# Artemarius/cuda-gaussian-splatting

Measured on AMD Instinct MI355X. Metric: fwd+bwd Mpixels/s @1080p, 1M Gaussians, SH3, higher is better.
Workload: dtype f32

## Files before the change

cuda-gaussian-splatting_amd/csrc/cugs_raster_common.h:

```cpp
#pragma once

#include "cugs_gaussian_math.h"
#include "cugs_blend_cull.h"

#include <type_traits>

#define CUGS_REC_F4 3

struct RasterGeom {
    int width, height, ntx, ntiles;
    float bg0, bg1, bg2;
};

struct RasterSrc {
    const int32_t* tile_ranges;
    const int32_t* gidx;
    const float* packed;
    const float* means_2d;
    const float* cov_2d_inv;
    const float* rgb;
    const float* opa;
    const uint4* tile_order;
};

template <typename F>
static inline void cugs_with_bool(bool flag, F&& f) {
    if (flag) f(std::true_type{});
    else f(std::false_type{});
}

__device__ __forceinline__ void cugs_stage_cull(const float4& r0, float4& r1, float tile_cx, float tile_cy) {
    r1.z = cugs_cull_limit(r0.x, r0.y, r0.z, r0.w, r1.x, r1.z, tile_cx, tile_cy);
}
__device__ __forceinline__ bool may_touch_quad(float4 r0, float4 r1, float qx0, float qy0,
                                               float wx, float wy) {
    return cugs_cull_may_touch(r0.x, r0.y, r0.z, r0.w, r1.x, r1.z, qx0, qy0, wx, wy);
}

template <bool PACKED, bool DEPTH = false>
__device__ __forceinline__ int stage_record(const RasterSrc& s, int li, int end, float4* s_rec, float tile_cx,
                                            float tile_cy, const float* __restrict__ depths = nullptr) {
    if (li >= end) return -1;
    const int g = s.gidx[li];
    float4 r0, r1, r2;
    if (PACKED) {
        const float4* src = reinterpret_cast<const float4*>(s.packed + (int64_t)g * CUGS_PACKED_STRIDE);
        r0 = src[0]; r1 = src[1]; r2 = src[2];
    } else {
        const float a = s.cov_2d_inv[g * 3 + 0], c = s.cov_2d_inv[g * 3 + 2], o = s.opa[g];
        r0 = make_float4(s.means_2d[g * 2 + 0], s.means_2d[g * 2 + 1], a, s.cov_2d_inv[g * 3 + 1]);
        r1 = make_float4(c, o, (o >= (1.0f / 255.0f)) ? logf(255.0f * o) : -1.0f, 0.0f);
        r2 = make_float4(s.rgb[g * 3 + 0], 0.0f, s.rgb[g * 3 + 1], s.rgb[g * 3 + 2]);
    }
    r1.w = __int_as_float(g);
    cugs_stage_cull(r0, r1, tile_cx, tile_cy);
    if (DEPTH) r2.y = depths[g];
    s_rec[threadIdx.x * CUGS_REC_F4 + 0] = r0;
    s_rec[threadIdx.x * CUGS_REC_F4 + 1] = r1;
    s_rec[threadIdx.x * CUGS_REC_F4 + 2] = r2;
    return g;
}

struct ActiveRect { float x0, y0, wx, wy; };
__device__ __forceinline__ ActiveRect active_rect(unsigned long long active, float quad_cx, float quad_cy) {
    unsigned cols = (unsigned)active | (unsigned)(active >> 32);
    cols |= cols >> 16;
    cols |= cols >> 8;
    cols &= 0xFFu;
    const int x0 = __builtin_ctz(cols), x1 = 31 - __builtin_clz(cols);
    const int y0 = __builtin_ctzll(active) >> 3, y1 = (63 - __builtin_clzll(active)) >> 3;
    return ActiveRect{quad_cx + (float)x0, quad_cy + (float)y0, (float)(x1 - x0), (float)(y1 - y0)};
}

#define CUGS_HIT_GROUP 4
__device__ __forceinline__ unsigned cugs_pop_hit_desc(unsigned long long& mask) {
    const unsigned bit = 63u - (unsigned)__builtin_clzll(mask);
    mask &= ~(1ull << bit);
    return bit;
}
__device__ __forceinline__ unsigned cugs_pop_hit_asc(unsigned long long& mask) {
    const unsigned bit = (unsigned)__builtin_ctzll(mask);
    mask &= mask - 1ull;
    return bit;
}
__device__ __forceinline__ unsigned long long cugs_pop_hits4_desc(unsigned long long& mask, unsigned rec_base) {
    const unsigned r0 = rec_base + cugs_pop_hit_desc(mask) * CUGS_REC_F4;
    const unsigned r1 = rec_base + cugs_pop_hit_desc(mask) * CUGS_REC_F4;
    const unsigned r2 = rec_base + cugs_pop_hit_desc(mask) * CUGS_REC_F4;
    const unsigned r3 = rec_base + cugs_pop_hit_desc(mask) * CUGS_REC_F4;
    return (unsigned long long)(r0 | (r1 << 16)) | ((unsigned long long)(r2 | (r3 << 16)) << 32);
}
__device__ __forceinline__ int cugs_hit(unsigned long long hitrecs, int field) {
    return (int)((hitrecs >> (16 * field)) & 0xFFFFull);
}
__device__ __forceinline__ unsigned long long cugs_set_hit(unsigned long long hitrecs, int field, unsigned rec) {
    return (hitrecs & ~(0xFFFFull << (16 * field))) | ((unsigned long long)rec << (16 * field));
}

struct PixelEval { float dx, dy, gx, gy, e; };
__device__ __forceinline__ float pixel_alpha_raw(float pxf, float pyf, float mx, float my, float a, float b,
                                                 float c, float o, float open, PixelEval& r) {
    r.dx = pxf - mx;
    r.dy = pyf - my;
    r.gx = fmaf(a, r.dx, b * r.dy);
    r.gy = fmaf(b, r.dx, c * r.dy);
    const float q = fmaf(r.dx, r.gx, r.dy * r.gy);
    r.e = cugs_blend_exp_q(q);
    const float gate = fmaf(q, 0x1p127f, 1.0f);
    return __builtin_fminf(__builtin_fminf((o * open) * r.e, 0.99f), gate);
}
__device__ __forceinline__ float pixel_alpha(float pxf, float pyf, float mx, float my, float a, float b,
                                             float c, float o, float open, PixelEval& r) {
    const float alpha = pixel_alpha_raw(pxf, pyf, mx, my, a, b, c, o, open, r);
    return (alpha < (1.0f / 255.0f)) ? 0.0f : alpha;
}


__device__ __forceinline__ float sat_fma(float a, float b, float c) {
    return __builtin_amdgcn_fmed3f(fmaf(a, b, c), 0.0f, 1.0f);
}
__device__ __forceinline__ float sat_add(float a, float b) { return __builtin_amdgcn_fmed3f(a + b, 0.0f, 1.0f); }
__device__ __forceinline__ float sat_mul(float a, float b) { return __builtin_amdgcn_fmed3f(a * b, 0.0f, 1.0f); }

#define CUGS_ALPHA_MIN_PRED 0x1.01010p-8f
__device__ __forceinline__ float passes_alpha_min(float x) {
    return sat_fma(x, 0x1p32f, -CUGS_ALPHA_MIN_PRED * 0x1p32f);
}
__device__ __forceinline__ float below_alpha_cap(float x) { return sat_fma(x, -0x1p32f, 0.99f * 0x1p32f); }

__device__ __forceinline__ int reduce9t_slot(int lane) {
    if (lane & 3) return -1;
    const int bank = (lane >> 2) & 3, row = lane >> 4;
    const int perm[4] = {0, 2, 1, 3};
    if (row == 0) return perm[bank];
    if (row == 1) return bank == 3 ? 8 : 4 + perm[bank];
    if (row == 2 && bank == 0) return 7;
    return -1;
}

__device__ __forceinline__ float reduce9t(float cA, float cB, float v2, float v3, float v4, float v5, float v6,
                                          float v8, float v7) {
    float a0, a1, a2, a3, a4, b0, b1, b2, d;
    asm volatile(
        "s_nop 1\n\t"
        "v_add_f32_dpp %0, %10, %9 row_mirror row_mask:0xf bank_mask:0xf\n\t"
        "v_add_f32_dpp %1, %11, %11 row_mirror row_mask:0xf bank_mask:0x3\n\t"
        "v_add_f32_dpp %1, %12, %12 row_mirror row_mask:0xf bank_mask:0xc\n\t"
        "v_add_f32_dpp %2, %13, %13 row_mirror row_mask:0xf bank_mask:0x3\n\t"
        "v_add_f32_dpp %2, %14, %14 row_mirror row_mask:0xf bank_mask:0xc\n\t"
        "v_add_f32_dpp %3, %15, %15 row_mirror row_mask:0xf bank_mask:0x3\n\t"
        "v_add_f32_dpp %3, %16, %16 row_mirror row_mask:0xf bank_mask:0xc\n\t"
        "v_add_f32_dpp %4, %17, %17 row_mirror row_mask:0xf bank_mask:0xf\n\t"
        "v_add_f32_dpp %5, %0, %0 row_half_mirror row_mask:0xf bank_mask:0x5\n\t"
        "v_add_f32_dpp %5, %1, %1 row_half_mirror row_mask:0xf bank_mask:0xa\n\t"
        "v_add_f32_dpp %7, %4, %4 row_half_mirror row_mask:0xf bank_mask:0xf\n\t"
        "v_add_f32_dpp %6, %2, %2 row_half_mirror row_mask:0xf bank_mask:0x5\n\t"
        "v_add_f32_dpp %6, %3, %3 row_half_mirror row_mask:0xf bank_mask:0xa\n\t"
        "v_mov_b32 %8, %7\n\t"
        "s_nop 1\n\t"
        "v_permlane16_swap_b32 %5, %6\n\t"
        "v_permlane16_swap_b32 %7, %8\n\t"
        "v_add_f32 %5, %5, %6\n\t"
        "v_add_f32 %7, %7, %8\n\t"
        "s_nop 1\n\t"
        "v_permlane32_swap_b32 %5, %7\n\t"
        "v_add_f32 %8, %5, %7\n\t"
        "s_nop 1\n\t"
        "v_add_f32_dpp %8, %8, %8 quad_perm:[1,0,3,2] row_mask:0xf bank_mask:0xf\n\t"
        "s_nop 1\n\t"
        "v_add_f32_dpp %8, %8, %8 quad_perm:[2,3,0,1] row_mask:0xf bank_mask:0xf\n\t"
        : "=&v"(a0), "=&v"(a1), "=&v"(a2), "=&v"(a3), "=&v"(a4), "=&v"(b0), "=&v"(b1), "=&v"(b2), "=&v"(d)
        : "v"(cA), "v"(cB), "v"(v2), "v"(v3), "v"(v4), "v"(v5), "v"(v6), "v"(v8), "v"(v7));
    return d;
}

template <int CTRL>
__device__ __forceinline__ float dpp_mov(float v) {
    return __builtin_bit_cast(float, __builtin_amdgcn_update_dpp(0, __builtin_bit_cast(int, v), CTRL, 0xF, 0xF, false));
}
template <int CTRL>
__device__ __forceinline__ float xchg_add(bool side, float a, float b) {
    return (side ? b : a) + dpp_mov<CTRL>(side ? a : b);
}

__device__ __forceinline__ int reduce9r16_slot(int lane) {
    const int r = lane & 15, bank = r >> 2;
    const int perm[4] = {0, 2, 1, 3};
    if ((r & 3) == 0) return perm[bank];
    if ((r & 3) == 2) return bank == 3 ? 8 : 4 + perm[bank];
    if (r == 1) return 7;
    return -1;
}

__device__ __forceinline__ float reduce_r16_tail(float b0, float b1, float b2, int lane) {
    const bool s1 = (lane & 2) != 0, s0 = (lane & 1) != 0;
    const float c0 = xchg_add<0x4E>(s1, b0, b1);
    const float c1 = b2 + dpp_mov<0x4E>(b2);
    return xchg_add<0xB1>(s0, c0, c1);
}

__device__ __forceinline__ float reduce9r16(float cA, float cB, float v2, float v3, float v4, float v5, float v6,
                                            float v8, float v7, int lane) {
    float a0, a1, a2, a3, a4, b0, b1, b2;
    asm volatile(
        "s_nop 1\n\t"
        "v_add_f32_dpp %0, %9, %8 row_mirror row_mask:0xf bank_mask:0xf\n\t"
        "v_add_f32_dpp %1, %10, %10 row_mirror row_mask:0xf bank_mask:0x3\n\t"
        "v_add_f32_dpp %1, %11, %11 row_mirror row_mask:0xf bank_mask:0xc\n\t"
        "v_add_f32_dpp %2, %12, %12 row_mirror row_mask:0xf bank_mask:0x3\n\t"
        "v_add_f32_dpp %2, %13, %13 row_mirror row_mask:0xf bank_mask:0xc\n\t"
        "v_add_f32_dpp %3, %14, %14 row_mirror row_mask:0xf bank_mask:0x3\n\t"
        "v_add_f32_dpp %3, %15, %15 row_mirror row_mask:0xf bank_mask:0xc\n\t"
        "v_add_f32_dpp %4, %16, %16 row_mirror row_mask:0xf bank_mask:0xf\n\t"
        "v_add_f32_dpp %5, %0, %0 row_half_mirror row_mask:0xf bank_mask:0x5\n\t"
        "v_add_f32_dpp %5, %1, %1 row_half_mirror row_mask:0xf bank_mask:0xa\n\t"
        "v_add_f32_dpp %7, %4, %4 row_half_mirror row_mask:0xf bank_mask:0xf\n\t"
        "v_add_f32_dpp %6, %2, %2 row_half_mirror row_mask:0xf bank_mask:0x5\n\t"
        "v_add_f32_dpp %6, %3, %3 row_half_mirror row_mask:0xf bank_mask:0xa\n\t"
        "s_nop 1\n\t"
        : "=&v"(a0), "=&v"(a1), "=&v"(a2), "=&v"(a3), "=&v"(a4), "=&v"(b0), "=&v"(b1), "=&v"(b2)
        : "v"(cA), "v"(cB), "v"(v2), "v"(v3), "v"(v4), "v"(v5), "v"(v6), "v"(v8), "v"(v7));
    return reduce_r16_tail(b0, b1, b2, lane);
}

__device__ __forceinline__ int reduce10r16_slot(int lane) {
    return ((lane & 15) == 9) ? 9 : reduce9r16_slot(lane);
}

__device__ __forceinline__ float reduce10r16(float cA, float cB, float v2, float v3, float v4, float v5, float v6,
                                             float v8, float v7, float v9, int lane) {
    float a0, a1, a2, a3, a4, b0, b1, b2;
    asm volatile(
        "s_nop 1\n\t"
        "v_add_f32_dpp %0, %9, %8 row_mirror row_mask:0xf bank_mask:0xf\n\t"
        "v_add_f32_dpp %1, %10, %10 row_mirror row_mask:0xf bank_mask:0x3\n\t"
        "v_add_f32_dpp %1, %11, %11 row_mirror row_mask:0xf bank_mask:0xc\n\t"
        "v_add_f32_dpp %2, %12, %12 row_mirror row_mask:0xf bank_mask:0x3\n\t"
        "v_add_f32_dpp %2, %13, %13 row_mirror row_mask:0xf bank_mask:0xc\n\t"
        "v_add_f32_dpp %3, %14, %14 row_mirror row_mask:0xf bank_mask:0x3\n\t"
        "v_add_f32_dpp %3, %15, %15 row_mirror row_mask:0xf bank_mask:0xc\n\t"
        "v_add_f32_dpp %4, %16, %16 row_mirror row_mask:0xf bank_mask:0x3\n\t"
        "v_add_f32_dpp %4, %17, %17 row_mirror row_mask:0xf bank_mask:0xc\n\t"
        "v_add_f32_dpp %5, %0, %0 row_half_mirror row_mask:0xf bank_mask:0x5\n\t"
        "v_add_f32_dpp %5, %1, %1 row_half_mirror row_mask:0xf bank_mask:0xa\n\t"
        "v_add_f32_dpp %7, %4, %4 row_half_mirror row_mask:0xf bank_mask:0xf\n\t"
        "v_add_f32_dpp %6, %2, %2 row_half_mirror row_mask:0xf bank_mask:0x5\n\t"
        "v_add_f32_dpp %6, %3, %3 row_half_mirror row_mask:0xf bank_mask:0xa\n\t"
        "s_nop 1\n\t"
        : "=&v"(a0), "=&v"(a1), "=&v"(a2), "=&v"(a3), "=&v"(a4), "=&v"(b0), "=&v"(b1), "=&v"(b2)
        : "v"(cA), "v"(cB), "v"(v2), "v"(v3), "v"(v4), "v"(v5), "v"(v6), "v"(v8), "v"(v7), "v"(v9));
    return reduce_r16_tail(b0, b1, b2, lane);
}

__device__ __forceinline__ int reduce12ar16_slot(int lane, bool with9) {
    const int r = lane & 15;
    if (r == 5) return 10;
    if (r == 13) return 11;
    if (r == 9) return with9 ? 9 : -1;
    return reduce9r16_slot(lane);
}

__device__ __forceinline__ float reduce12ar16(float cA, float cB, float v2, float v3, float v4, float v5, float v6,
                                              float v8, float v7, float v9, float v10, float v11, int lane) {
    float a0, a1, a2, a3, a4, a5, b0, b1, b2;
    asm volatile(
        "s_nop 1\n\t"
        "v_add_f32_dpp %0, %10, %9 row_mirror row_mask:0xf bank_mask:0xf\n\t"
        "v_add_f32_dpp %1, %11, %11 row_mirror row_mask:0xf bank_mask:0x3\n\t"
        "v_add_f32_dpp %1, %12, %12 row_mirror row_mask:0xf bank_mask:0xc\n\t"
        "v_add_f32_dpp %2, %13, %13 row_mirror row_mask:0xf bank_mask:0x3\n\t"
        "v_add_f32_dpp %2, %14, %14 row_mirror row_mask:0xf bank_mask:0xc\n\t"
        "v_add_f32_dpp %3, %15, %15 row_mirror row_mask:0xf bank_mask:0x3\n\t"
        "v_add_f32_dpp %3, %16, %16 row_mirror row_mask:0xf bank_mask:0xc\n\t"
        "v_add_f32_dpp %4, %17, %17 row_mirror row_mask:0xf bank_mask:0x3\n\t"
        "v_add_f32_dpp %4, %18, %18 row_mirror row_mask:0xf bank_mask:0xc\n\t"
        "v_add_f32_dpp %5, %19, %19 row_mirror row_mask:0xf bank_mask:0x3\n\t"
        "v_add_f32_dpp %5, %20, %20 row_mirror row_mask:0xf bank_mask:0xc\n\t"
        "v_add_f32_dpp %6, %0, %0 row_half_mirror row_mask:0xf bank_mask:0x5\n\t"
        "v_add_f32_dpp %6, %1, %1 row_half_mirror row_mask:0xf bank_mask:0xa\n\t"
        "v_add_f32_dpp %8, %4, %4 row_half_mirror row_mask:0xf bank_mask:0x5\n\t"
        "v_add_f32_dpp %8, %5, %5 row_half_mirror row_mask:0xf bank_mask:0xa\n\t"
        "v_add_f32_dpp %7, %2, %2 row_half_mirror row_mask:0xf bank_mask:0x5\n\t"
        "v_add_f32_dpp %7, %3, %3 row_half_mirror row_mask:0xf bank_mask:0xa\n\t"
        "s_nop 1\n\t"
        : "=&v"(a0), "=&v"(a1), "=&v"(a2), "=&v"(a3), "=&v"(a4), "=&v"(a5), "=&v"(b0), "=&v"(b1), "=&v"(b2)
        : "v"(cA), "v"(cB), "v"(v2), "v"(v3), "v"(v4), "v"(v5), "v"(v6), "v"(v8), "v"(v7), "v"(v9), "v"(v10), "v"(v11));
    return reduce_r16_tail(b0, b1, b2, lane);
}

__device__ __forceinline__ int reduce12r16_slot(int lane) {
    const int r = lane & 15;
    if ((r & 3) == 3) return -1;
    return ((r & 1) ? 2 : ((r >> 1) & 1)) + 3 * ((r >> 2) & 1) + 6 * ((r >> 3) & 1);
}

__device__ __forceinline__ float reduce12r16(const float (&v)[12], int lane) {
    const bool s3 = (lane & 8) != 0, s2 = (lane & 4) != 0;
    float u[6], w[3];
#pragma unroll
    for (int k = 0; k < 6; ++k) u[k] = xchg_add<0x140>(s3, v[k], v[k + 6]);
#pragma unroll
    for (int k = 0; k < 3; ++k) w[k] = xchg_add<0x141>(s2, u[k], u[k + 3]);
    return reduce_r16_tail(w[0], w[1], w[2], lane);
}
```

cuda-gaussian-splatting_amd/csrc/raster_backward.hip:

```cpp
#include "cugs_raster_common.h"

#include <cstdlib>

#ifdef CUGS_DEV
bool cugs_dev_backward_stats();
#endif

namespace {

#define CUGS_BWD_HITS 4
static_assert(CUGS_BWD_HITS == CUGS_HIT_GROUP, "a hit group is one flush");
#ifndef CUGS_BWD_ABS_WAVES
#define CUGS_BWD_ABS_WAVES 7
#endif
#ifndef CUGS_BWD_HSTRIDE
#define CUGS_BWD_HSTRIDE 64
#endif

template <bool PACKED, bool WIDE, bool STATS, bool DEPTH = false, bool ABS = false>
__global__ __launch_bounds__(CUGS_BLOCK) __attribute__((amdgpu_waves_per_eu(ABS ? CUGS_BWD_ABS_WAVES : (DEPTH ? 7 : 8))))
void k_raster_backward(RasterGeom geo, RasterSrc src,
                                                                const float* __restrict__ dL_dcolor,
                                                                const float* __restrict__ final_T,
                                                                const int32_t* __restrict__ n_contrib,
                                                                float* __restrict__ grad_accum, int64_t stats_row,
                                                                const float* __restrict__ depths,
                                                                const float* __restrict__ dL_ddepth_map,
                                                                const float* __restrict__ dL_dalpha) {
    __shared__ float4 s_rec[CUGS_BLOCK * CUGS_REC_F4];
    __shared__ float2 s_contrib[4][CUGS_BWD_HITS][CUGS_BWD_HSTRIDE];

#ifdef CUGS_DEV
    const bool no_atomics = stats_row == -2;
#else
    constexpr bool no_atomics = false;
#endif
    unsigned tile;
    int range_start, range_end;
    if (src.tile_order) {
        const uint4 rec = src.tile_order[blockIdx.x];
        tile = rec.x; range_start = (int)rec.y; range_end = (int)rec.z;
    } else {
        tile = cugs_blend_tile(blockIdx.x, (unsigned)geo.ntx, (unsigned)(geo.ntiles / geo.ntx));
        range_start = src.tile_ranges[tile * 2 + 0];
        range_end = src.tile_ranges[tile * 2 + 1];
    }
    const int tile_x = (int)(tile % (unsigned)geo.ntx), tile_y = (int)(tile / (unsigned)geo.ntx);
    const int tid = threadIdx.x, wave = tid >> 6, lane = tid & 63;
    const int quad_x = tile_x * CUGS_TILE + (wave & 1) * 8, quad_y = tile_y * CUGS_TILE + (wave >> 1) * 8;
    const int px = quad_x + (lane & 7), py = quad_y + (lane >> 3);
    const bool inside = (px < geo.width) && (py < geo.height);
    const float pxf = (float)px + 0.5f, pyf = (float)py + 0.5f;
    const float qx0 = (float)quad_x + 0.5f, qy0 = (float)quad_y + 0.5f;
    const float tile_cx = (float)(tile_x * CUGS_TILE + CUGS_TILE / 2), tile_cy = (float)(tile_y * CUGS_TILE + CUGS_TILE / 2);

    const int num_in_range = range_end - range_start;
    const int num_batches = (num_in_range + CUGS_BLOCK - 1) / CUGS_BLOCK;

    const int pix = py * geo.width + px;
    float T = inside ? final_T[pix] : 0.0f;
    const int max_contrib = inside ? n_contrib[pix] : 0;
    float dC0 = 0.0f, dC1 = 0.0f, dC2 = 0.0f;
    if (inside) {
        dC0 = dL_dcolor[pix * 3 + 0];
        dC1 = dL_dcolor[pix * 3 + 1];
        dC2 = dL_dcolor[pix * 3 + 2];
    }
    float dDp = 0.0f;
    if (DEPTH && inside && dL_ddepth_map) dDp = dL_ddepth_map[pix];
    const int h2 = lane >> 4, g2i = lane & 15;
    const int gx0 = quad_x + (g2i & 1) * 4, gy = quad_y + (g2i >> 1);
    const float px2 = (float)gx0 + 0.5f, py2 = (float)gy + 0.5f;
    const bool side = (lane & 8) != 0;
    float eA[4], eB[4], e2[4], eZ[4];
#pragma unroll
    for (int i = 0; i < 4; ++i) {
        float r = 0.0f, gg = 0.0f, bb = 0.0f, zz = 0.0f;
        if (gx0 + i < geo.width && gy < geo.height) {
            const int pq = gy * geo.width + gx0 + i, q = pq * 3;
            r = dL_dcolor[q + 0]; gg = dL_dcolor[q + 1]; bb = dL_dcolor[q + 2];
            if (DEPTH && dL_ddepth_map) zz = dL_ddepth_map[pq];
        }
        eA[i] = side ? gg : r; eB[i] = side ? r : gg; e2[i] = bb; eZ[i] = zz;
    }
    const int slot2 = ABS ? reduce12ar16_slot(lane, DEPTH) : DEPTH ? reduce10r16_slot(lane) : reduce9r16_slot(lane);
    const unsigned slot_off = (unsigned)(slot2 < 0 ? 0 : slot2) * 4u;
    unsigned long long hitrecs = 0ull;

    float D = fmaf(dC2, T * geo.bg2, fmaf(dC1, T * geo.bg1, dC0 * (T * geo.bg0)));
    if (DEPTH && inside && dL_dalpha) D = fmaf(-T, dL_dalpha[pix], D);
    float rem = (inside && max_contrib > 0) ? (float)max_contrib : -1.0f;
    bool wave_done = (__ballot(rem >= 0.0f) == 0ull);
    int pending = 0;
    unsigned st_steps = 0, st_contrib = 0, st_lanes = 0, st_batches = 0, st_tested = 0, st_open = 0;

    auto flush = [&](int cnt) {
        const int rec = (int)((hitrecs >> (16 * h2)) & 0xFFFFull);
        const float4* c4 = reinterpret_cast<const float4*>(&s_contrib[wave][h2][g2i * 4]);
        const float4 p01 = c4[0], p23 = c4[1];
        float4 head;
        if (ABS) {
            head = s_rec[rec];
        } else {
            const float2 m = *reinterpret_cast<const float2*>(&s_rec[rec]);
            head = make_float4(m.x, m.y, 0.0f, 0.0f);
        }
        const float2 mean = make_float2(head.x, head.y);
        const float4 tail = s_rec[rec + 1];
        const float dy = py2 - mean.y;
        const float dx0 = px2 - mean.x, dx1 = dx0 + 1.0f, dx2 = dx0 + 2.0f, dx3 = dx0 + 3.0f;
        float t = p01.y * dx0;
        float A = p01.y, M1 = t, Mxx = t * dx0;
        float RA = p01.x * eA[0], RB = p01.x * eB[0], R2 = p01.x * e2[0];
        t = p01.w * dx1; A += p01.w; M1 += t; Mxx = fmaf(t, dx1, Mxx);
        RA = fmaf(p01.z, eA[1], RA); RB = fmaf(p01.z, eB[1], RB); R2 = fmaf(p01.z, e2[1], R2);
        t = p23.y * dx2; A += p23.y; M1 += t; Mxx = fmaf(t, dx2, Mxx);
        RA = fmaf(p23.x, eA[2], RA); RB = fmaf(p23.x, eB[2], RB); R2 = fmaf(p23.x, e2[2], R2);
        t = p23.w * dx3; A += p23.w; M1 += t; Mxx = fmaf(t, dx3, Mxx);
        RA = fmaf(p23.z, eA[3], RA); RB = fmaf(p23.z, eB[3], RB); R2 = fmaf(p23.z, e2[3], R2);
        const float oA = tail.y * A;
        M1 *= tail.y; Mxx *= tail.y;
        const float M1y = dy * oA, Myy = dy * M1y, Mxy = dy * M1;
        float total;
        if (ABS) {
            const float bdy = head.w * dy, cdy = tail.x * dy;
            float SX = fabsf(p01.y) * fabsf(fmaf(head.z, dx0, bdy));
            float SY = fabsf(p01.y) * fabsf(fmaf(head.w, dx0, cdy));
            SX = fmaf(fabsf(p01.w), fabsf(fmaf(head.z, dx1, bdy)), SX);
            SY = fmaf(fabsf(p01.w), fabsf(fmaf(head.w, dx1, cdy)), SY);
            SX = fmaf(fabsf(p23.y), fabsf(fmaf(head.z, dx2, bdy)), SX);
            SY = fmaf(fabsf(p23.y), fabsf(fmaf(head.w, dx2, cdy)), SY);
            SX = fmaf(fabsf(p23.w), fabsf(fmaf(head.z, dx3, bdy)), SX);
            SY = fmaf(fabsf(p23.w), fabsf(fmaf(head.w, dx3, cdy)), SY);
            const float ao = fabsf(tail.y);
            SX *= ao; SY *= ao;
            float RZ = 0.0f;
            if (DEPTH) {
                RZ = p01.x * eZ[0];
                RZ = fmaf(p01.z, eZ[1], RZ); RZ = fmaf(p23.x, eZ[2], RZ); RZ = fmaf(p23.z, eZ[3], RZ);
            }
            total = reduce12ar16(RA, RB, R2, A, M1, M1y, Mxx, Myy, Mxy, RZ, SX, SY, lane);
        } else if (DEPTH) {
            float RZ = p01.x * eZ[0];
            RZ = fmaf(p01.z, eZ[1], RZ); RZ = fmaf(p23.x, eZ[2], RZ); RZ = fmaf(p23.z, eZ[3], RZ);
            total = reduce10r16(RA, RB, R2, A, M1, M1y, Mxx, Myy, Mxy, RZ, lane);
        } else {
            total = reduce9r16(RA, RB, R2, A, M1, M1y, Mxx, Myy, Mxy, lane);
        }
        if (slot2 >= 0 && h2 < cnt && !no_atomics) {
            const int g = __float_as_int(tail.w);
            if (WIDE) {
                atomicAdd(grad_accum + (int64_t)g * CUGS_GRAD_STRIDE + slot2, total);
            } else {
                const unsigned off = ((unsigned)g << 6) + slot_off;
                atomicAdd(reinterpret_cast<float*>(reinterpret_cast<char*>(grad_accum) + off), total);
            }
        }
    };

    auto step = [&](const int rec, const int slot) __attribute__((always_inline)) {
        if (STATS) ++st_steps;
        const float4 g0 = s_rec[rec], g1 = s_rec[rec + 1], col = s_rec[rec + 2];
        const float o = g1.y;

        PixelEval e;
        const float alpha = pixel_alpha_raw(pxf, pyf, g0.x, g0.y, g0.z, g0.w, g1.x, o, 1.0f, e);
        const float passf = passes_alpha_min(alpha);
        const float k = sat_mul(passf, rem);
        rem -= passf;
        const float al = alpha * k;
        const float gk = k * below_alpha_cap(alpha);

        const float rcp = __builtin_amdgcn_rcpf(1.0f - al);
        T *= rcp;
        const float weight = al * T;
        float G = fmaf(dC2, col.w, fmaf(dC1, col.z, dC0 * col.x));
        if (DEPTH) G = fmaf(dDp, col.y, G);
        const float gate = fmaf(T, G, -(rcp * D)) * gk;
        D = fmaf(weight, G, D);
        if (STATS) {
            const unsigned long long lm = __ballot(k != 0.0f);
            if (lm) { ++st_contrib; st_lanes += __popcll(lm); st_open += __popcll(__ballot(rem >= 0.0f)); }
        }
        s_contrib[wave][slot][lane] = make_float2(weight, gate * e.e);
    };

    for (int batch = num_batches - 1; batch >= 0; --batch) {
        if (lane == 0) s_contrib[wave][0][0].x = wave_done ? 1.0f : 0.0f;
        __syncthreads();
        if (s_contrib[0][0][0].x * s_contrib[1][0][0].x * s_contrib[2][0][0].x * s_contrib[3][0][0].x != 0.0f) break;

        stage_record<PACKED, DEPTH>(src, range_start + batch * CUGS_BLOCK + tid, range_end, s_rec, tile_cx, tile_cy, depths);
        __syncthreads();

        if (STATS && !wave_done) ++st_batches;
        if (!wave_done) {
            const int batch_count = min(CUGS_BLOCK, num_in_range - batch * CUGS_BLOCK);
            const int nsub = (batch_count + CUGS_WAVE - 1) / CUGS_WAVE;
            for (int sub = nsub - 1; sub >= 0 && !wave_done; --sub) {
                const int j = sub * CUGS_WAVE + lane;
                const ActiveRect ar = active_rect(__ballot(rem >= 0.0f), qx0, qy0);
                bool hit = false;
                if (j < batch_count)
                    hit = may_touch_quad(s_rec[j * CUGS_REC_F4 + 0], s_rec[j * CUGS_REC_F4 + 1], ar.x0, ar.y0, ar.wx,
                                         ar.wy);
                unsigned long long mask = __ballot(hit);
                if (STATS) st_tested += min(CUGS_WAVE, batch_count - sub * CUGS_WAVE);
                const unsigned rec_sub = (unsigned)(sub * CUGS_WAVE * CUGS_REC_F4);
                while (pending + __popcll(mask) >= CUGS_BWD_HITS) {
                    if (pending == 0) {
                        hitrecs = cugs_pop_hits4_desc(mask, rec_sub);
                    } else {
                        do hitrecs = cugs_set_hit(hitrecs, pending, rec_sub + cugs_pop_hit_desc(mask) * CUGS_REC_F4);
                        while (++pending < CUGS_BWD_HITS);
                        pending = 0;
                    }
                    step(cugs_hit(hitrecs, 0), 0);
                    step(cugs_hit(hitrecs, 1), 1);
                    step(cugs_hit(hitrecs, 2), 2);
                    step(cugs_hit(hitrecs, 3), 3);
                    const bool closed = (__ballot(rem >= 0.0f) == 0ull);
                    flush(CUGS_BWD_HITS);
                    if (closed) { wave_done = true; mask = 0ull; break; }
                }
                while (mask != 0ull) {
                    hitrecs = cugs_set_hit(hitrecs, pending, rec_sub + cugs_pop_hit_desc(mask) * CUGS_REC_F4);
                    ++pending;
                }
            }
            if (pending) {
                for (int p = 0; p < pending; ++p) step(cugs_hit(hitrecs, p), p);
                if (__ballot(rem >= 0.0f) == 0ull) wave_done = true;
                flush(pending);
                pending = 0;
            }
        }
    }
    if (STATS && lane == 0) {
        float* st = grad_accum + (int64_t)stats_row * CUGS_GRAD_STRIDE;
        atomicAdd(&st[0], (float)st_steps); atomicAdd(&st[1], (float)st_contrib); atomicAdd(&st[2], (float)st_lanes);
        atomicAdd(&st[3], (float)st_batches); atomicAdd(&st[4], (float)st_tested); atomicAdd(&st[5], (float)num_batches);
        atomicAdd(&st[7], (float)st_open);
    }
}

template <bool PACKED, bool DEPTH = false, bool ABS = false>
__global__ __launch_bounds__(CUGS_BLOCK) void k_unpack_grads(int64_t n, const float* __restrict__ acc,
                                                             const float* __restrict__ packed,
                                                             const float* __restrict__ cov_2d_inv,
                                                             float* __restrict__ dL_drgb,
                                                             float* __restrict__ dL_dopa,
                                                             float* __restrict__ dL_dmeans,
                                                             float* __restrict__ dL_dcov,
                                                             float* __restrict__ dL_ddepths,
                                                             float* __restrict__ dL_dmeans_abs) {
    const int64_t i = (int64_t)blockIdx.x * CUGS_BLOCK + threadIdx.x;
    if (i >= n) return;
    const float4* row = reinterpret_cast<const float4*>(acc + i * CUGS_GRAD_STRIDE);
    const float4 r0 = row[0], r1 = row[1];
    float r2;
    if (ABS) {
        const float4 w = row[2];
        r2 = w.x;
        if (DEPTH) dL_ddepths[i] = w.y;
        *reinterpret_cast<float2*>(dL_dmeans_abs + i * 2) = make_float2(w.z, w.w);
    } else if (DEPTH) {
        const float2 w89 = *reinterpret_cast<const float2*>(acc + i * CUGS_GRAD_STRIDE + 8);
        r2 = w89.x;
        dL_ddepths[i] = w89.y;
    } else {
        r2 = acc[i * CUGS_GRAD_STRIDE + 8];
    }
    float a, b, c;
    if (PACKED) {
        const float4* rec = reinterpret_cast<const float4*>(packed + i * CUGS_PACKED_STRIDE);
        const float4 p0 = rec[0];
        a = p0.z; b = p0.w; c = rec[1].x;
    } else {
        a = cov_2d_inv[i * 3 + 0]; b = cov_2d_inv[i * 3 + 1]; c = cov_2d_inv[i * 3 + 2];
    }
    dL_drgb[i * 3 + 0] = r0.x; dL_drgb[i * 3 + 1] = r0.y; dL_drgb[i * 3 + 2] = r0.z;
    dL_dopa[i] = r0.w;
    const GradMoments m{r1.x, r1.y, r1.z, r1.w, r2};
    const Grad2D g = grads_from_moments(m, a, b, c);
    dL_dmeans[i * 2 + 0] = g.mx; dL_dmeans[i * 2 + 1] = g.my;
    dL_dcov[i * 3 + 0] = g.a; dL_dcov[i * 3 + 1] = g.b; dL_dcov[i * 3 + 2] = g.c;
}

}

extern "C" int cugs_rasterize_backward_opts(int width, int height, const float background_host[3],
                                            const int32_t* tile_ranges, const int32_t* gaussian_indices,
                                            const float* means_2d, const float* cov_2d_inv, const float* rgb,
                                            const float* opacities_act, const float* packed,
                                            const float* dL_dcolor, const float* final_T,
                                            const int32_t* n_contrib, int64_t n, float* grad_accum,
                                            float* dL_drgb, float* dL_dopacity_act, float* dL_dmeans_2d,
                                            float* dL_dcov_2d_inv, const cugs_blend_backward_opts* opts, void* stream) {
    const cugs_blend_backward_opts o = opts ? *opts : cugs_blend_backward_opts{};
    const bool depth_map = o.depths || o.dL_ddepth_map || o.dL_dalpha;
    const bool abs_grad = o.abs_grad != 0;
    if (width < 0 || height < 0 || n < 0 || !background_host) return CUGS_EINVAL;
    if (n == 0) return 0;
    if (!grad_accum) return CUGS_EINVAL;
    if ((reinterpret_cast<uintptr_t>(grad_accum) & 63u) != 0) return CUGS_EALIGN;
    const int n_soa = (dL_drgb != nullptr) + (dL_dopacity_act != nullptr) + (dL_dmeans_2d != nullptr) +
                      (dL_dcov_2d_inv != nullptr);
    if (n_soa != 0 && n_soa != 4) return CUGS_EINVAL;
    if (depth_map && (n_soa == 4) != (o.dL_ddepths != nullptr)) return CUGS_EINVAL;
    if (!depth_map && o.dL_ddepths) return CUGS_EINVAL;
    if (abs_grad && (n_soa == 4) != (o.dL_dmeans_2d_abs != nullptr)) return CUGS_EINVAL;
    if (n_soa == 4 && !packed && !cov_2d_inv) return CUGS_EINVAL;
    if (packed && !cugs_aligned16(packed)) return CUGS_EALIGN;
    if (o.tile_order && !cugs_aligned16(o.tile_order)) return CUGS_EALIGN;
    hipStream_t st = static_cast<hipStream_t>(stream);
    int64_t rows = n;
#ifdef CUGS_DEV
    const bool stats = cugs_dev_backward_stats();
    if (stats) rows = n + 1;
#endif
    if (!o.prezeroed || rows != n)
        CUGS_RETURN_IF_HIP(hipMemsetAsync(grad_accum, 0, sizeof(float) * CUGS_GRAD_STRIDE * (size_t)rows, st));

    const int ntx = (width + CUGS_TILE - 1) / CUGS_TILE, nty = (height + CUGS_TILE - 1) / CUGS_TILE;
    if (ntx > 0 && nty > 0 && gaussian_indices) {
        if (!tile_ranges || !dL_dcolor || !final_T || !n_contrib) return CUGS_EINVAL;
        if (!packed && (!means_2d || !cov_2d_inv || !rgb || !opacities_act)) return CUGS_EINVAL;
        if (depth_map && !o.depths) return CUGS_EINVAL;
        if ((int64_t)width * height > 2147483647ll / 3) return CUGS_EOVERFLOW;
        RasterGeom geo{width, height, ntx, ntx * nty, background_host[0], background_host[1], background_host[2]};
        RasterSrc src{tile_ranges, gaussian_indices, packed, means_2d, cov_2d_inv, rgb, opacities_act, reinterpret_cast<const uint4*>(o.tile_order)};
        const bool wide = rows > (int64_t(1) << 26);
        int64_t stats_arg = n;
#ifdef CUGS_DEV
        if (const char* e = std::getenv("CUGS_BWD_NO_ATOMICS")) if (e[0] == '1') stats_arg = -2;
#endif
        const auto launch = [&](auto* kernel) {
            hipLaunchKernelGGL(kernel, dim3(geo.ntiles), dim3(CUGS_BLOCK), 0, st, geo, src, dL_dcolor, final_T, n_contrib,
                               grad_accum, stats_arg, o.depths, o.dL_ddepth_map, o.dL_dalpha);
        };
#ifdef CUGS_DEV
        if (stats && !depth_map && !abs_grad)
            cugs_with_bool(packed != nullptr, [&](auto P) { launch(k_raster_backward<P(), true, true>); });
        else
#endif
        cugs_with_bool(packed != nullptr, [&](auto P) { cugs_with_bool(wide, [&](auto W) {
            cugs_with_bool(depth_map, [&](auto D) { cugs_with_bool(abs_grad, [&](auto A) {
                launch(k_raster_backward<P(), W(), false, D(), A()>);
            }); });
        }); });
        CUGS_LAUNCH_CHECK();
    }
    if (n_soa == 4) {
        const dim3 grid((unsigned)((n + CUGS_BLOCK - 1) / CUGS_BLOCK));
        cugs_with_bool(packed != nullptr, [&](auto P) { cugs_with_bool(depth_map, [&](auto D) {
            cugs_with_bool(abs_grad, [&](auto A) {
                hipLaunchKernelGGL((k_unpack_grads<P(), D(), A()>), grid, dim3(CUGS_BLOCK), 0, st, n, grad_accum, packed,
                                   cov_2d_inv, dL_drgb, dL_dopacity_act, dL_dmeans_2d, dL_dcov_2d_inv, o.dL_ddepths,
                                   o.dL_dmeans_2d_abs);
            });
        }); });
        CUGS_LAUNCH_CHECK();
    }
    return 0;
}

extern "C" int cugs_rasterize_backward(int width, int height, const float background_host[3],
                                       const int32_t* tile_ranges, const int32_t* gaussian_indices,
                                       const float* means_2d, const float* cov_2d_inv, const float* rgb,
                                       const float* opacities_act, const float* packed,
                                       const float* dL_dcolor, const float* final_T,
                                       const int32_t* n_contrib, int64_t n, float* grad_accum,
                                       float* dL_drgb, float* dL_dopacity_act, float* dL_dmeans_2d,
                                       float* dL_dcov_2d_inv, void* stream) {
    return cugs_rasterize_backward_opts(width, height, background_host, tile_ranges, gaussian_indices, means_2d, cov_2d_inv,
                                        rgb, opacities_act, packed, dL_dcolor, final_T, n_contrib, n, grad_accum, dL_drgb,
                                        dL_dopacity_act, dL_dmeans_2d, dL_dcov_2d_inv, nullptr, stream);
}

#ifdef CUGS_DEV
namespace {
__global__ void k_dbg_reduce9(const float* __restrict__ in, float* __restrict__ out, int* __restrict__ slots) {
    const int l = threadIdx.x;
    const bool side = (l & 8) != 0;
    const float v0 = in[0 * 64 + l], v1 = in[1 * 64 + l];
    out[l] = reduce9t(side ? v1 : v0, side ? v0 : v1, in[2 * 64 + l], in[3 * 64 + l], in[4 * 64 + l], in[5 * 64 + l],
                      in[6 * 64 + l], in[8 * 64 + l], in[7 * 64 + l]);
    slots[l] = reduce9t_slot(l);
}
__global__ void k_dbg_reduce9r16(const float* __restrict__ in, float* __restrict__ out, int* __restrict__ slots) {
    const int l = threadIdx.x;
    const bool side = (l & 8) != 0;
    const float v0 = in[0 * 64 + l], v1 = in[1 * 64 + l];
    out[l] = reduce9r16(side ? v1 : v0, side ? v0 : v1, in[2 * 64 + l], in[3 * 64 + l], in[4 * 64 + l], in[5 * 64 + l],
                        in[6 * 64 + l], in[8 * 64 + l], in[7 * 64 + l], l);
    slots[l] = reduce9r16_slot(l);
}
__global__ void k_dbg_reduce10r16(const float* __restrict__ in, float* __restrict__ out, int* __restrict__ slots) {
    const int l = threadIdx.x;
    const bool side = (l & 8) != 0;
    const float v0 = in[0 * 64 + l], v1 = in[1 * 64 + l];
    out[l] = reduce10r16(side ? v1 : v0, side ? v0 : v1, in[2 * 64 + l], in[3 * 64 + l], in[4 * 64 + l], in[5 * 64 + l],
                         in[6 * 64 + l], in[8 * 64 + l], in[7 * 64 + l], in[9 * 64 + l], l);
    slots[l] = reduce10r16_slot(l);
}
__global__ void k_dbg_reduce12ar16(const float* __restrict__ in, float* __restrict__ out, int* __restrict__ slots,
                                   int* __restrict__ slots_nodepth) {
    const int l = threadIdx.x;
    const bool side = (l & 8) != 0;
    const float v0 = in[0 * 64 + l], v1 = in[1 * 64 + l];
    out[l] = reduce12ar16(side ? v1 : v0, side ? v0 : v1, in[2 * 64 + l], in[3 * 64 + l], in[4 * 64 + l], in[5 * 64 + l],
                          in[6 * 64 + l], in[8 * 64 + l], in[7 * 64 + l], in[9 * 64 + l], in[10 * 64 + l], in[11 * 64 + l],
                          l);
    slots[l] = reduce12ar16_slot(l, true);
    slots_nodepth[l] = reduce12ar16_slot(l, false);
}
__global__ void k_dbg_rcp(const float* __restrict__ in, float* __restrict__ out, int n) {
    const int i = blockIdx.x * blockDim.x + threadIdx.x;
    if (i < n) out[i] = __builtin_amdgcn_rcpf(in[i]);
}
__global__ void k_dbg_blend_exp(const float* __restrict__ q, float* __restrict__ out, int n) {
    const int i = blockIdx.x * blockDim.x + threadIdx.x;
    if (i < n) out[i] = cugs_blend_exp_q(q[i]);
}
__global__ void k_dbg_may_touch_quad(int n, const float* __restrict__ in, const unsigned long long* __restrict__ masks,
                                     int* __restrict__ hit, unsigned long long* __restrict__ pass,
                                     float* __restrict__ rect) {
    const int i = blockIdx.x * blockDim.x + threadIdx.x;
    if (i >= n) return;
    const float* c = in + (int64_t)i * 8;
    alignas(16) float rec[CUGS_PACKED_STRIDE];
    write_packed(rec, 0, c[0], c[1], Sym2{c[2], c[3], c[4]}, 0.0f, 0.0f, 0.0f, c[5]);
    const float4 r0 = reinterpret_cast<const float4*>(rec)[0];
    float4 r1 = reinterpret_cast<const float4*>(rec)[1];
    const int quad_x = (int)c[6], quad_y = (int)c[7];
    cugs_stage_cull(r0, r1, (float)((quad_x & ~(CUGS_TILE - 1)) + CUGS_TILE / 2), (float)((quad_y & ~(CUGS_TILE - 1)) + CUGS_TILE / 2));
    const float qx0 = (float)quad_x + 0.5f, qy0 = (float)quad_y + 0.5f;
    const unsigned long long active = masks[i];
    const ActiveRect ar = active_rect(active, qx0, qy0);
    hit[i] = may_touch_quad(r0, r1, ar.x0, ar.y0, ar.wx, ar.wy) ? 1 : 0;
    unsigned long long p = 0ull;
    for (int l = 0; l < 64; ++l) {
        const float pxf = (float)(quad_x + (l & 7)) + 0.5f, pyf = (float)(quad_y + (l >> 3)) + 0.5f;
        const float open = ((active >> l) & 1ull) ? 1.0f : 0.0f;
        PixelEval e;
        const float alpha = pixel_alpha_raw(pxf, pyf, r0.x, r0.y, r0.z, r0.w, r1.x, r1.y, open, e);
        if (passes_alpha_min(alpha) != 0.0f) p |= 1ull << l;
    }
    pass[i] = p;
    rect[(int64_t)i * 4 + 0] = ar.x0 - qx0; rect[(int64_t)i * 4 + 1] = ar.y0 - qy0;
    rect[(int64_t)i * 4 + 2] = ar.wx; rect[(int64_t)i * 4 + 3] = ar.wy;
}
bool g_dev_backward_stats = false;
}
bool cugs_dev_backward_stats() { return g_dev_backward_stats; }
extern "C" int cugsdbg_backward_stats(int on) { g_dev_backward_stats = (on != 0); return 0; }
extern "C" int cugsdbg_reduce9(const float* in, float* out, int* slots, void* stream) {
    hipLaunchKernelGGL(k_dbg_reduce9, dim3(1), dim3(64), 0, static_cast<hipStream_t>(stream), in, out, slots);
    CUGS_LAUNCH_CHECK();
    return 0;
}
extern "C" int cugsdbg_reduce9r16(const float* in, float* out, int* slots, void* stream) {
    hipLaunchKernelGGL(k_dbg_reduce9r16, dim3(1), dim3(64), 0, static_cast<hipStream_t>(stream), in, out, slots);
    CUGS_LAUNCH_CHECK();
    return 0;
}
extern "C" int cugsdbg_reduce10r16(const float* in, float* out, int* slots, void* stream) {
    hipLaunchKernelGGL(k_dbg_reduce10r16, dim3(1), dim3(64), 0, static_cast<hipStream_t>(stream), in, out, slots);
    CUGS_LAUNCH_CHECK();
    return 0;
}
extern "C" int cugsdbg_reduce12ar16(const float* in, float* out, int* slots, int* slots_nodepth, void* stream) {
    hipLaunchKernelGGL(k_dbg_reduce12ar16, dim3(1), dim3(64), 0, static_cast<hipStream_t>(stream), in, out, slots,
                       slots_nodepth);
    CUGS_LAUNCH_CHECK();
    return 0;
}
extern "C" int cugsdbg_blend_exp_q(const float* q, float* out, int n, void* stream) {
    hipLaunchKernelGGL(k_dbg_blend_exp, dim3((n + 255) / 256), dim3(256), 0, static_cast<hipStream_t>(stream), q, out, n);
    CUGS_LAUNCH_CHECK();
    return 0;
}
extern "C" int cugsdbg_rcp(const float* in, float* out, int n, void* stream) {
    hipLaunchKernelGGL(k_dbg_rcp, dim3((n + 255) / 256), dim3(256), 0, static_cast<hipStream_t>(stream), in, out, n);
    CUGS_LAUNCH_CHECK();
    return 0;
}
extern "C" int cugsdbg_may_touch_quad(int n, const float* in, const unsigned long long* masks, int* hit,
                                      unsigned long long* pass, float* rect, void* stream) {
    if (n <= 0) return n == 0 ? 0 : CUGS_EINVAL;
    hipLaunchKernelGGL(k_dbg_may_touch_quad, dim3((n + 255) / 256), dim3(256), 0, static_cast<hipStream_t>(stream), n, in,
                       masks, hit, pass, rect);
    CUGS_LAUNCH_CHECK();
    return 0;
}
#endif
```

Before: 2839.

## Prefetch first backward batch alongside per-pixel loads and realign batches to range end

The backward raster kernel now fetches the first batch's Gaussian index and record before the pixel-state loads. The per-pixel and per-group gradient loads become unconditional, using clamped addresses and selects, so all of this memory latency overlaps in the prologue. Batches are now counted from range_end, so the first processed batch is full and the trailing partial batch sits at range_start. The first batch skips the completion-vote barrier, and empty tiles return early. The cost is extra live registers across the prologue and redundant loads for out-of-image pixels. A new stats counter tracks how many batches were staged.

```diff
diff --git a/cuda-gaussian-splatting_amd/csrc/cugs_raster_common.h b/cuda-gaussian-splatting_amd/csrc/cugs_raster_common.h
--- a/cuda-gaussian-splatting_amd/csrc/cugs_raster_common.h
+++ b/cuda-gaussian-splatting_amd/csrc/cugs_raster_common.h
@@ -38,11 +38,8 @@
 }
 
 template <bool PACKED, bool DEPTH = false>
-__device__ __forceinline__ int stage_record(const RasterSrc& s, int li, int end, float4* s_rec, float tile_cx,
+__device__ __forceinline__ void stage_fetch(const RasterSrc& s, int g, float4& r0, float4& r1, float4& r2, float tile_cx,
                                             float tile_cy, const float* __restrict__ depths = nullptr) {
-    if (li >= end) return -1;
-    const int g = s.gidx[li];
-    float4 r0, r1, r2;
     if (PACKED) {
         const float4* src = reinterpret_cast<const float4*>(s.packed + (int64_t)g * CUGS_PACKED_STRIDE);
         r0 = src[0]; r1 = src[1]; r2 = src[2];
@@ -55,9 +52,20 @@
     r1.w = __int_as_float(g);
     cugs_stage_cull(r0, r1, tile_cx, tile_cy);
     if (DEPTH) r2.y = depths[g];
+}
+__device__ __forceinline__ void stage_store(float4* s_rec, const float4& r0, const float4& r1, const float4& r2) {
     s_rec[threadIdx.x * CUGS_REC_F4 + 0] = r0;
     s_rec[threadIdx.x * CUGS_REC_F4 + 1] = r1;
     s_rec[threadIdx.x * CUGS_REC_F4 + 2] = r2;
+}
+template <bool PACKED, bool DEPTH = false>
+__device__ __forceinline__ int stage_record(const RasterSrc& s, int li, int end, float4* s_rec, float tile_cx,
+                                            float tile_cy, const float* __restrict__ depths = nullptr) {
+    if (li >= end) return -1;
+    const int g = s.gidx[li];
+    float4 r0, r1, r2;
+    stage_fetch<PACKED, DEPTH>(s, g, r0, r1, r2, tile_cx, tile_cy, depths);
+    stage_store(s_rec, r0, r1, r2);
     return g;
 }
 
diff --git a/cuda-gaussian-splatting_amd/csrc/raster_backward.hip b/cuda-gaussian-splatting_amd/csrc/raster_backward.hip
--- a/cuda-gaussian-splatting_amd/csrc/raster_backward.hip
+++ b/cuda-gaussian-splatting_amd/csrc/raster_backward.hip
@@ -55,17 +55,18 @@
     const float tile_cx = (float)(tile_x * CUGS_TILE + CUGS_TILE / 2), tile_cy = (float)(tile_y * CUGS_TILE + CUGS_TILE / 2);
 
     const int num_in_range = range_end - range_start;
+    if (num_in_range <= 0) return;
     const int num_batches = (num_in_range + CUGS_BLOCK - 1) / CUGS_BLOCK;
 
-    const int pix = py * geo.width + px;
-    float T = inside ? final_T[pix] : 0.0f;
-    const int max_contrib = inside ? n_contrib[pix] : 0;
-    float dC0 = 0.0f, dC1 = 0.0f, dC2 = 0.0f;
-    if (inside) {
-        dC0 = dL_dcolor[pix * 3 + 0];
-        dC1 = dL_dcolor[pix * 3 + 1];
-        dC2 = dL_dcolor[pix * 3 + 2];
-    }
+    const int g_first = src.gidx[min(max(range_start, range_end - CUGS_BLOCK) + tid, range_end - 1)];
+
+    const int pix = inside ? py * geo.width + px : 0;
+    const float T_ld = final_T[pix];
+    const int n_ld = n_contrib[pix];
+    const float c0_ld = dL_dcolor[pix * 3 + 0], c1_ld = dL_dcolor[pix * 3 + 1], c2_ld = dL_dcolor[pix * 3 + 2];
+    float T = inside ? T_ld : 0.0f;
+    const int max_contrib = inside ? n_ld : 0;
+    const float dC0 = inside ? c0_ld : 0.0f, dC1 = inside ? c1_ld : 0.0f, dC2 = inside ? c2_ld : 0.0f;
     float dDp = 0.0f;
     if (DEPTH && inside && dL_ddepth_map) dDp = dL_ddepth_map[pix];
     const int h2 = lane >> 4, g2i = lane & 15;
@@ -75,14 +76,16 @@
     float eA[4], eB[4], e2[4], eZ[4];
 #pragma unroll
     for (int i = 0; i < 4; ++i) {
-        float r = 0.0f, gg = 0.0f, bb = 0.0f, zz = 0.0f;
-        if (gx0 + i < geo.width && gy < geo.height) {
-            const int pq = gy * geo.width + gx0 + i, q = pq * 3;
-            r = dL_dcolor[q + 0]; gg = dL_dcolor[q + 1]; bb = dL_dcolor[q + 2];
-            if (DEPTH && dL_ddepth_map) zz = dL_ddepth_map[pq];
-        }
+        const bool in2 = gx0 + i < geo.width && gy < geo.height;
+        const int pq = in2 ? gy * geo.width + gx0 + i : 0, q = pq * 3;
+        const float r_ld = dL_dcolor[q + 0], g_ld = dL_dcolor[q + 1], b_ld = dL_dcolor[q + 2];
+        const float r = in2 ? r_ld : 0.0f, gg = in2 ? g_ld : 0.0f, bb = in2 ? b_ld : 0.0f;
+        float zz = 0.0f;
+        if (DEPTH && in2 && dL_ddepth_map) zz = dL_ddepth_map[pq];
         eA[i] = side ? gg : r; eB[i] = side ? r : gg; e2[i] = bb; eZ[i] = zz;
     }
+    float4 st0, st1, st2;
+    stage_fetch<PACKED, DEPTH>(src, g_first, st0, st1, st2, tile_cx, tile_cy, depths);
     const int slot2 = ABS ? reduce12ar16_slot(lane, DEPTH) : DEPTH ? reduce10r16_slot(lane) : reduce9r16_slot(lane);
     const unsigned slot_off = (unsigned)(slot2 < 0 ? 0 : slot2) * 4u;
     unsigned long long hitrecs = 0ull;
@@ -92,7 +95,7 @@
     float rem = (inside && max_contrib > 0) ? (float)max_contrib : -1.0f;
     bool wave_done = (__ballot(rem >= 0.0f) == 0ull);
     int pending = 0;
-    unsigned st_steps = 0, st_contrib = 0, st_lanes = 0, st_batches = 0, st_tested = 0, st_open = 0;
+    unsigned st_steps = 0, st_contrib = 0, st_lanes = 0, st_batches = 0, st_tested = 0, st_open = 0, st_staged = 0;
 
     auto flush = [&](int cnt) {
         const int rec = (int)((hitrecs >> (16 * h2)) & 0xFFFFull);
@@ -185,17 +188,14 @@
         s_contrib[wave][slot][lane] = make_float2(weight, gate * e.e);
     };
 
-    for (int batch = num_batches - 1; batch >= 0; --batch) {
-        if (lane == 0) s_contrib[wave][0][0].x = wave_done ? 1.0f : 0.0f;
-        __syncthreads();
-        if (s_contrib[0][0][0].x * s_contrib[1][0][0].x * s_contrib[2][0][0].x * s_contrib[3][0][0].x != 0.0f) break;
-
-        stage_record<PACKED, DEPTH>(src, range_start + batch * CUGS_BLOCK + tid, range_end, s_rec, tile_cx, tile_cy, depths);
-        __syncthreads();
-
+    stage_store(s_rec, st0, st1, st2);
+    __syncthreads();
+    if (STATS) ++st_staged;
+    for (int batch = 0;;) {
+        const int hi = range_end - batch * CUGS_BLOCK, lo = max(range_start, hi - CUGS_BLOCK);
         if (STATS && !wave_done) ++st_batches;
         if (!wave_done) {
-            const int batch_count = min(CUGS_BLOCK, num_in_range - batch * CUGS_BLOCK);
+            const int batch_count = hi - lo;
             const int nsub = (batch_count + CUGS_WAVE - 1) / CUGS_WAVE;
             for (int sub = nsub - 1; sub >= 0 && !wave_done; --sub) {
                 const int j = sub * CUGS_WAVE + lane;
@@ -235,12 +235,21 @@
                 pending = 0;
             }
         }
+        if (++batch == num_batches) break;
+        if (lane == 0) s_contrib[wave][0][0].x = wave_done ? 1.0f : 0.0f;
+        __syncthreads();
+        if (s_contrib[0][0][0].x * s_contrib[1][0][0].x * s_contrib[2][0][0].x * s_contrib[3][0][0].x != 0.0f) break;
+
+        const int nhi = range_end - batch * CUGS_BLOCK;
+        stage_record<PACKED, DEPTH>(src, max(range_start, nhi - CUGS_BLOCK) + tid, nhi, s_rec, tile_cx, tile_cy, depths);
+        __syncthreads();
+        if (STATS) ++st_staged;
     }
     if (STATS && lane == 0) {
         float* st = grad_accum + (int64_t)stats_row * CUGS_GRAD_STRIDE;
         atomicAdd(&st[0], (float)st_steps); atomicAdd(&st[1], (float)st_contrib); atomicAdd(&st[2], (float)st_lanes);
         atomicAdd(&st[3], (float)st_batches); atomicAdd(&st[4], (float)st_tested); atomicAdd(&st[5], (float)num_batches);
-        atomicAdd(&st[7], (float)st_open);
+        atomicAdd(&st[6], (float)st_staged); atomicAdd(&st[7], (float)st_open);
     }
 }
 
```

Result: no change. 2849 (median of 6 runs) (+0.4%).
